# khimansusinha/Distributed-sorting-with-fault-tolerance

Measured on AMD Instinct MI355X. Metric: sorted keys/sec (int32, 2^30 keys), higher is better.
Workload: dtype int32; 1 GPU; C2-style single-GPU sort of 1073741824 uniform int32 keys (BASELINE metric size); tile 8192 keys, 0 merge passes; keys=1073741824, parallelism=1 GPU

## Files before the change

### distributed-sorting-with-fault-tolerance_amd/csrc/dsort_internal.h

```cpp
#pragma once

#include <hip/hip_runtime.h>
#include <stdint.h>
#include <stddef.h>

#include <atomic>
#include <mutex>
#include <string>
#include <utility>
#include <vector>

#include "dsort.h"

struct ncclComm;
namespace dsort {
class TxSeq;
}

namespace dsort {

constexpr int kMaxLogF = 5;
constexpr int kMaxF = 1 << kMaxLogF;

struct GroupK {
// ... 79 lines not shown
    void mark_at(int i, hipStream_t s) {
        if (!ok || i >= kMax) return;
        ok = (ev[i].h || hipEventCreate(&ev[i].h) == hipSuccess) && hipEventRecord(ev[i], s) == hipSuccess;
        if (ok) n = i + 1;
    }
    int count() const { return ok ? n : 0; }
    bool complete(int events) const { return count() == events; }
    int wait_last(dsort_ctx *ctx) const;
    int elapsed(dsort_ctx *ctx, int a, int b, double *ms) const;
};

}

struct dsort_opts {
    int64_t buckets = -1;
    int64_t bucket_keys = 1 << 20;
    static constexpr int64_t BUCKET_OS_DEFAULT = 128;
    int64_t bucket_os = BUCKET_OS_DEFAULT;
    int64_t max_logf = -1;
    int64_t kill_after_pass = -1;
    int64_t stage_timing = 1;
    int64_t kill_in_exchange = -1;
    int64_t comm_timeout_ms = 0;
    int64_t test_hold_exchange = 0;
    int64_t test_fail_exchange = -1;
    int64_t test_tile_cap = 0;
    int64_t test_wave_fence = 0;
    int64_t sub_keys = -1;
    int64_t sub_os = -1;
    int64_t sub_gather = 1;
    int64_t argsort_wide = 0;
    int64_t test_fail_leg = -1;
    int64_t topk_path = -1;
};

struct dsort_ctx {
    using DevBuf = dsort::DevBuf;
    using HostBuf = dsort::HostBuf;
    using Event = dsort::Event;
    using Stream = dsort::Stream;
    using LegClock = dsort::LegClock;

    dsort_opts opt;
    int nested = 0;
    int stages_done = 0;
    std::atomic<int> abort_req{0};
    std::mutex comm_mu;
    int device = 0;
    std::string err;

    Stream stream;
    Stream side;
    Stream xs;

    Event groups_ev;
    Event bucket_ev;
    Event sub_ev;
    Event side_ev;
    Event ready_ev;
    Event done_ev;
    Event a64_mm_ev;
    Event xev[3];
    Event ev[dsort::kStageEvents];
    static constexpr int kMaxKev = 128;
    Event kev[kMaxKev];
    LegClock pairs_clk;
// ... 37 lines not shown
    DevBuf gat_rep;
    DevBuf gat_back;
    DevBuf gat_small;
    HostBuf gat_host;
    DevBuf bucket;
    HostBuf bucket_host;
    DevBuf sub;
    DevBuf sub_alt;
    DevBuf stmp;
    HostBuf sub_host;
    hipStream_t done_stream = nullptr;
    bool done_pending = false;
    DevBuf tfb;
    DevBuf text_status;
    DevBuf red;
    HostBuf red_host;
    ncclComm *comm = nullptr;
    bool has_transport = false;
    dsort_transport transport = {};
    dsort::TxSeq *tx = nullptr;
    HostBuf xfer;
    HostBuf xfer2;
    DevBuf fence;
    HostBuf fence_host;
    int nranks = 1;
    int rank = 0;
    DevBuf local;
    DevBuf recv;
    DevBuf recv2;
    DevBuf small;
    HostBuf small_host;
    DevBuf bxs;
    const uint32_t *bk_hot = nullptr;
    int ev_off = 0;
    int ev_done = dsort::kEvLocalDone;
    bool poll_waits = false;
    double poll_deadline = 0.0;
    hipStream_t poll_stream = nullptr;
    std::vector<void *> dev_later, host_later;
    uint64_t deferred_n = 0;
    unsigned ev_mask = 0;
    hipStream_t last_stream = nullptr;
    int kev_used = 0;
    bool ev_ok = false;
    bool ev_created = false;
    dsort_stats stats = {};
};

namespace dsort {

__device__ __forceinline__ uint32_t wave_incl_sum(uint32_t v) {
    v += (uint32_t)__builtin_amdgcn_update_dpp(0, (int)v, 0x111, 0xF, 0xF, false);
    v += (uint32_t)__builtin_amdgcn_update_dpp(0, (int)v, 0x112, 0xF, 0xF, false);
    v += (uint32_t)__builtin_amdgcn_update_dpp(0, (int)v, 0x114, 0xF, 0xF, false);
    v += (uint32_t)__builtin_amdgcn_update_dpp(0, (int)v, 0x118, 0xF, 0xF, false);
    v += (uint32_t)__builtin_amdgcn_update_dpp(0, (int)v, 0x142, 0xA, 0xF, false);
    v += (uint32_t)__builtin_amdgcn_update_dpp(0, (int)v, 0x143, 0xC, 0xF, false);
    return v;
}

inline dsort_stats fresh_stats() {
    dsort_stats s{};
    s.first_level_map = -1;
    return s;
}

// ... 73 lines not shown
```

### distributed-sorting-with-fault-tolerance_amd/csrc/dsort_sub.h

```cpp
#pragma once
#include <hip/hip_runtime.h>
#include <stdint.h>

#include "dsort_bucket.h"

namespace dsort {
namespace sb {

constexpr int SB_T = 256;
constexpr int SB_MAXS = 1024;
constexpr int SB_SLOTB = 10;
constexpr int SB_SLOTS = 1 << SB_SLOTB;
constexpr int SB_ST = 4;
template <typename T> constexpr int SB_KPT = sizeof(T) == 4 ? 16 : 8;
template <typename T> constexpr int SB_SUB = SB_T * SB_KPT<T>;
template <typename T> constexpr int SB_CH = SB_ST * SB_SUB<T>;

struct BInfo {
    uint64_t start;
    uint64_t soff;
    uint32_t len;
    uint32_t nsub;
    uint32_t ns;
    uint32_t c0, c1;
// ... 6 lines not shown
    uint32_t len;
    uint32_t b;
    uint32_t boff;
    uint32_t pad;
};

__device__ __forceinline__ uint64_t bucket_src_pos(const BInfo &b, const Chunk *ch, uint64_t p) {
    if (!b.multi) return b.start + p;
    uint32_t lo = b.c0, hi = b.c1 - 1;
    while (lo < hi) {
        const uint32_t mid = (lo + hi + 1) >> 1;
        if (ch[mid].boff <= p) lo = mid;
        else hi = mid - 1;
    }
    return ch[lo].start + (p - ch[lo].boff);
}

template <typename T>
__device__ __forceinline__ Chunk chunk_of(const Chunk *ch, const BInfo *bi, uint32_t c) {
    if (ch) return ch[c];
    const uint64_t o = (uint64_t)c * SB_CH<T>, len = bi[0].len;
    return Chunk{bi[0].start + o, (uint32_t)(len - o < (uint64_t)SB_CH<T> ? len - o : (uint64_t)SB_CH<T>), 0u,
                 (uint32_t)o, 0u};
}

template <typename T> struct KeyU;
template <> struct KeyU<int32_t> { using U = uint32_t; };
template <> struct KeyU<int64_t> { using U = uint64_t; };

template <typename T>
struct SlotFn {
    T klo;
    uint32_t sh;
    uint32_t pad;
};

template <typename T>
__host__ __device__ __forceinline__ uint32_t slot_of(T key, T klo, uint32_t sh) {
    using U = typename KeyU<T>::U;
    const U d = key < klo ? (U)0 : (U)((U)key - (U)klo);
    const U s = d >> sh;
    return s > (U)(SB_SLOTS - 1) ? (uint32_t)(SB_SLOTS - 1) : (uint32_t)s;
}

template <typename T> struct Spl;
template <> struct __attribute__((aligned(8))) Spl<int32_t> {
    int32_t k;
    uint32_t p;
};
template <> struct __attribute__((aligned(16))) Spl<int64_t> {
    int64_t k;
    uint32_t p, pad;
};

template <typename T>
__device__ __forceinline__ bool below(const Spl<T> &s, T key, uint32_t pos) {
    return s.k < key || (s.k == key && s.p <= pos);
}

constexpr uint32_t SB_ONEKEY = 0x8000u;
template <typename T>
__device__ __forceinline__ int sub_pick(const Spl<T> *spl, uint32_t r, const Spl<T> &a, const Spl<T> &b, T key,
                                        uint32_t pos) {
    int lo = (int)(r & 0x7FFF);
    const int hi = (int)(r >> 16);
    if (r & SB_ONEKEY) {
        if (key != a.k) return key < a.k ? lo : hi;
        if (pos < a.p) return lo;
        const Spl<T> z = spl[hi - 1];
        if (pos >= z.p) return hi;
        const float f = (float)((pos * 2654435761u) >> 8) * 0x1p-24f;
        const int jj = (int)(f * (float)(hi - lo - 1));
        return lo + 1 + (jj < hi - lo - 2 ? jj : hi - lo - 2);
    }
    const int j = lo + (lo < hi && below<T>(a, key, pos) ? 1 + (lo + 1 < hi && below<T>(b, key, pos)) : 0);
    if (j < lo + 2 || j >= hi) return j;
    lo = j;
    int h = hi;
    while (lo < h) {
        const int mid = (lo + h) >> 1;
        if (below<T>(spl[mid], key, pos)) lo = mid + 1;
        else h = mid;
    }
    return lo;
}
template <typename T>
__device__ __forceinline__ int sub_of(const Spl<T> *spl, const uint32_t *rng, T klo, uint32_t sh, T key,
                                      uint32_t pos) {
    const uint32_t r = rng[slot_of<T>(key, klo, sh)];
    const int lo = (int)(r & 0x7FFF), hi = (int)(r >> 16);
    Spl<T> a{}, b{};
    if (lo < hi) a = spl[lo];
    if (lo + 1 < hi) b = spl[lo + 1];
    return sub_pick<T>(spl, r, a, b, key, pos);
}

constexpr uint32_t SB_RUN = 8;
constexpr uint32_t SB_SMP_CH = 1024;
__host__ __device__ __forceinline__ uint32_t sample_run(const BInfo &b) { return b.single || b.ns % SB_RUN ? 1u : SB_RUN; }
__host__ __device__ __forceinline__ uint64_t sample_run_pos(const BInfo &b, uint32_t run, uint64_t r) {
    const uint64_t nr = b.ns / run;
    const uint64_t p = ((2 * r + 1) * b.len) / (2 * nr);
    return p + run > b.len ? b.len - run : p;
}
__host__ __device__ __forceinline__ uint64_t sample_pos(const BInfo &b, uint64_t k) {
    const uint32_t run = sample_run(b);
    return sample_run_pos(b, run, k / run) + k % run;
}
template <typename T>
__global__ void __launch_bounds__(SB_T) sb_sample_kernel(const T *__restrict__ src, const BInfo *__restrict__ bi,
                                                         const Chunk *__restrict__ ch, T *__restrict__ smp,
                                                         int64_t *__restrict__ cmp) {
    const BInfo b = bi[blockIdx.x];
    auto put = [&](uint64_t k, T key) {
        const uint64_t g = b.soff + k;
        smp[g] = key;
        if constexpr (sizeof(T) == 4) cmp[g] = (int64_t)((uint64_t)(int64_t)key << 32 | (uint32_t)g);
    };
    if (sample_run(b) == SB_RUN && !b.multi) {
#pragma unroll 2
// ... 39 lines not shown

template <typename T>
__device__ __forceinline__ uint32_t lower_bound_k(const T *a, uint32_t n, T k) {
    uint32_t lo = 0, hi = n;
    while (lo < hi) {
        const uint32_t mid = (lo + hi) >> 1;
        if (a[mid] < k) lo = mid + 1;
        else hi = mid;
    }
    return lo;
}
template <typename T>
__device__ __forceinline__ uint32_t upper_bound_k(const T *a, uint32_t n, T k) {
    uint32_t lo = 0, hi = n;
    while (lo < hi) {
        const uint32_t mid = (lo + hi) >> 1;
        if (!(k < a[mid])) lo = mid + 1;
        else hi = mid;
    }
    return lo;
}

__global__ void __launch_bounds__(SB_T) sb_rank_kernel(const int64_t *__restrict__ smp, const int64_t *__restrict__ srt,
                                                       const BInfo *__restrict__ bi, int64_t *__restrict__ cmp) {
    const BInfo b = bi[blockIdx.x];
    for (uint32_t k = threadIdx.x; k < b.ns; k += SB_T) {
        const uint64_t g = b.soff + k;
        const uint64_t lo = b.soff + lower_bound_k<int64_t>(srt + b.soff, b.ns, smp[g]);
        cmp[g] = (int64_t)(lo << 32 | (uint32_t)g);
    }
}

template <typename T>
__global__ void __launch_bounds__(SB_MAXS) sb_splitter_kernel(const int64_t *__restrict__ cmp, const T *__restrict__ smp,
                                                              const BInfo *__restrict__ bi, const Chunk *__restrict__ ch,
                                                              int os, int SS,
                                                              Spl<T> *__restrict__ spl, uint32_t *__restrict__ rng,
                                                              SlotFn<T> *__restrict__ sfn, uint32_t *__restrict__ stot) {
    using U = typename KeyU<T>::U;
    __shared__ uint32_t sslot[SB_MAXS];
    __shared__ T skey[SB_MAXS];
    const BInfo b = bi[blockIdx.x];
    const int tid = threadIdx.x;
    if (stot)
        for (int j = tid; j < SS; j += SB_MAXS) stot[(uint64_t)blockIdx.x * SS + j] = 0;
    const int nspl = (int)b.nsub - 1;
    T klo = 0;
    uint32_t sh = 0;
    if (nspl > 0) {
        const int64_t *cm = cmp + b.soff;
        klo = smp[(uint32_t)cm[0]];
        const U span = (U)((U)smp[(uint32_t)cm[b.ns - 1]] - (U)klo);
        while (sh < 8 * sizeof(T) && (span >> sh) >= (U)SB_SLOTS) ++sh;
        if (tid < nspl) {
            const uint32_t g = (uint32_t)cm[(uint32_t)(tid + 1) * (uint32_t)os - 1];
            const T K = smp[g];
            Spl<T> sp{};
            sp.k = K;
            sp.p = (uint32_t)bucket_src_pos(b, ch, sample_pos(b, g - b.soff));
            spl[(uint64_t)blockIdx.x * SS + tid] = sp;
            sslot[tid] = slot_of<T>(K, klo, sh);
            skey[tid] = K;
        }
    }
    __syncthreads();
    for (int s = tid; s < SB_SLOTS; s += SB_MAXS) {
        uint32_t lo = 0, hi = (uint32_t)(nspl > 0 ? nspl : 0);
        while (lo < hi) {
            const uint32_t mid = (lo + hi) >> 1;
            if (sslot[mid] < (uint32_t)s) lo = mid + 1;
            else hi = mid;
        }
        uint32_t lo2 = lo, hi2 = (uint32_t)(nspl > 0 ? nspl : 0);
        while (lo2 < hi2) {
            const uint32_t mid = (lo2 + hi2) >> 1;
            if (sslot[mid] <= (uint32_t)s) lo2 = mid + 1;
            else hi2 = mid;
        }
        const bool one = lo2 >= lo + 3 && skey[lo] == skey[lo2 - 1];
        rng[(uint64_t)blockIdx.x * SB_SLOTS + s] = lo | (one ? SB_ONEKEY : 0u) | (lo2 << 16);
    }
    if (tid == 0) sfn[blockIdx.x] = SlotFn<T>{klo, sh, 0};
}

template <typename T>
__device__ __forceinline__ void load_sub_tables(const BInfo &b, uint32_t bid, int SS, const Spl<T> *spl_g,
                                                const uint32_t *rng_g, Spl<T> *spl, uint32_t *rng) {
    const int nspl = (int)b.nsub - 1;
    for (int j = threadIdx.x; j < nspl; j += blockDim.x) spl[j] = spl_g[(uint64_t)bid * SS + j];
    for (int s = threadIdx.x; s < SB_SLOTS; s += blockDim.x) rng[s] = rng_g[(uint64_t)bid * SB_SLOTS + s];
}

template <typename T>
__global__ void __launch_bounds__(SB_T) sb_hist_kernel(const T *__restrict__ src, const Chunk *__restrict__ ch,
                                                       const BInfo *__restrict__ bi, int SS,
                                                       const Spl<T> *__restrict__ spl_g,
                                                       const uint32_t *__restrict__ rng_g,
                                                       const SlotFn<T> *__restrict__ sfn,
                                                       uint32_t *__restrict__ counts) {
    __shared__ Spl<T> spl[SB_MAXS + 1];
    __shared__ uint32_t rng[SB_SLOTS];
    __shared__ uint32_t hist[SB_MAXS];
    const Chunk c = chunk_of<T>(ch, bi, blockIdx.x);
    const BInfo b = bi[c.b];
    uint32_t *out = counts + (uint64_t)blockIdx.x * SS;
    if (b.nsub == 1) {
        if (threadIdx.x == 0) out[0] = c.len;
        return;
    }
    load_sub_tables<T>(b, c.b, SS, spl_g, rng_g, spl, rng);
    for (int j = threadIdx.x; j < (int)b.nsub; j += SB_T) hist[j] = 0;
    const SlotFn<T> f = sfn[c.b];
    __syncthreads();
    constexpr int UN = 8;
#pragma unroll 1
// ... 375 lines not shown
#define SBST(k)                                            \
    do {                                                   \
        const uint64_t t1_ = __builtin_amdgcn_s_memtime(); \
        st_acc[k] = t1_ - st_t0;                           \
        st_t0 = t1_;                                       \
    } while (0)
#else
#define SBST(k) \
    do {        \
    } while (0)
#endif
    const uint32_t cid = sb_chunk_order(blockIdx.x, gridDim.x);
    const Chunk c = ch[cid];
    const BInfo b = bi[c.b];
    uint32_t *pc = pref + (uint64_t)cid * (SS + 1);
    const int tid = threadIdx.x, lane = tid & 63, w = tid >> 6;
    const int ns = (int)b.nsub;
    if (ns == 1) {
        if (tid == 0) {
            pc[0] = 0;
            pc[1] = c.len;
            if (stot) atomicAdd(&stot[(uint64_t)c.b * SS], c.len);
        }
        return;
    }
    const uint32_t m = 0;
    T *src = buf + c.start;
    T key[KPT];
#pragma unroll
    for (int k = 0; k < KPT; ++k) {
        const uint32_t s = tid + k * LT;
        key[k] = s - m < c.len ? src[s] : T(0);
    }
    load_sub_tables<T>(b, c.b, SS, spl_g, rng_g, spl, rng);
#pragma unroll
    for (int q = 0; q < PER; ++q) hist[PER * tid + q] = 0;
    const SlotFn<T> f = sfn[c.b];
    const bool hotf = hotp != nullptr && *hotp != 0;
    __syncthreads();
    SBST(0);
    uint32_t pk[KPT];
    constexpr int G = sizeof(T) == 4 ? SB_G32 : SB_G64;
    const bool whole = c.len == (uint32_t)CHL;
    if constexpr (G == 1) {
        if (hotf) {
#pragma unroll
            for (int k = 0; k < KPT; ++k) {
                const uint32_t s = tid + k * LT;
                const bool act = s - m < c.len;
                const int j = act ? sub_of<T>(spl, rng, f.klo, f.sh, key[k], (uint32_t)(c.start + s - m)) : 0;
                pk[k] = (uint32_t)j | bk::bucket_bump<true>(hist, j, act) << 10;
            }
        } else if (whole) {
#pragma unroll
            for (int k = 0; k < KPT; ++k) {
                const uint32_t s = tid + k * LT;
                if ((k > 0 && k + 1 < KPT) || s - m < c.len) {
                    const int j = sub_of<T>(spl, rng, f.klo, f.sh, key[k], (uint32_t)(c.start + s - m));
                    pk[k] = (uint32_t)j | atomicAdd(&hist[j], 1u) << 10;
                }
            }
        } else
#pragma unroll
        for (int k = 0; k < KPT; ++k) {
            const uint32_t s = tid + k * LT;
            if (s - m < c.len) {
                const int j = sub_of<T>(spl, rng, f.klo, f.sh, key[k], (uint32_t)(c.start + s - m));
                pk[k] = (uint32_t)j | atomicAdd(&hist[j], 1u) << 10;
            }
        }
    } else {
#pragma unroll
    for (int g0 = 0; g0 < KPT; g0 += G) {
        uint32_t r[G];
        Spl<T> sa[G], sb[G];
#pragma unroll
        for (int u = 0; u < G; ++u)
// ... 170 lines not shown
```

### distributed-sorting-with-fault-tolerance_amd/csrc/dsort_wave.hip

```cpp
#include <hip/hip_runtime.h>

#include <stdint.h>

#include <algorithm>
#include <climits>
#include <ctime>
#include <sched.h>
#include <unistd.h>
#include <csignal>
#include <cstdlib>
#include <cstring>
#include <string>
#include <type_traits>
#include <vector>

#include "dsort_bucket.h"
#include "dsort_internal.h"
#include "dsort_tx.h"

#include <rocprofiler-sdk-roctx/roctx.h>
#include "dsort_part.h"
#include "dsort_sub.h"

namespace dsort {
// ... 1529 lines not shown
    uint32_t *rng;
    sb::SlotFn<T> *sfn;
    uint32_t *cnt, *offs;
    void *tt;
    sb::Ovf *ovf;
    uint32_t *num;
    bk::TileRef *stl;
    uint2 *pcs;
    FillSeg<T> *fill;
    uint32_t *stot;
    uint32_t *hn;
};
template <typename T>
static size_t sub_arena(const SubArgs<T> &a, const SubPlan<T> &p, uintptr_t base, SubArena<T> &A) {
    using namespace sb;
    const size_t B = (size_t)a.B, SS = (size_t)p.SS;
    uintptr_t at = base;
    auto take = [&](auto *&ptr, size_t bytes) {
        ptr = reinterpret_cast<std::remove_reference_t<decltype(ptr)>>(at);
        at += (bytes + 255) & ~(size_t)255;
    };
    take(A.bi, B * sizeof(BInfo));
    take(A.ch, p.nch * sizeof(Chunk));
    take(A.smp, p.nsmp * sizeof(T));
    take(A.cmp, p.nsmp * 8);
    take(A.srt, sizeof(T) == 8 ? p.nsmp * 8 : 0);
    take(A.spl, B * SS * sizeof(Spl<T>));
    take(A.rng, B * SB_SLOTS * 4);
    take(A.sfn, B * sizeof(SlotFn<T>));
    take(A.cnt, p.nch * (SS + 1) * 4);
    take(A.offs, p.local ? 0 : p.nch * SS * 4);
    take(A.tt, p.tmax * sizeof(GTile));
    take(A.ovf, p.nsubs * sizeof(Ovf));
    take(A.num, 8);
    take(A.stl, B * sizeof(bk::TileRef) + 16);
    take(A.pcs, p.local ? p.tcap * p.PS * sizeof(uint2) : 0);
    take(A.fill, a.pm || a.fill_keys ? B * sizeof(FillSeg<T>) : 0);
    take(A.stot, p.totals ? B * SS * 4 : 0);
    if (!p.totals) A.stot = nullptr;
    return at - base;
}

template <typename T>
static SubPlan<T> sub_plan(const dsort_opts &opt, const SubArgs<T> &a, uint64_t m_in, bool local, bool retry) {
    using namespace sb;
    const int B = a.B;
    const uint64_t *hb = a.hb;
    const uint8_t *pure = a.pure;
    const PieceMap<T> *pm = a.pm;
    SubPlan<T> p;
    uint64_t maxlen = 0;
    for (int b = 0; b < B; ++b)
        if (!pure[b]) maxlen = std::max<uint64_t>(maxlen, hb[b + 1] - hb[b]);
    const int TILE = sizeof(T) == 4 && maxlen > (uint64_t)SB_MAXS * TILE_OF<T> / 4 ? TILE_W<16> : TILE_OF<T>;
    const uint64_t m = opt.sub_keys < 0 && TILE != TILE_OF<T> ? (uint64_t)TILE / 8 : m_in;
    constexpr uint64_t ALIGN = KPC<T>;
    const bool asked_local = local;
    const uint64_t LCH = SB_LCH<T>;
    auto bucket_chunks = [&](int b, uint64_t ch) -> uint64_t {
        if (pure[b]) return 0;
        if (!pm) return ceil_div(hb[b + 1] - hb[b], ch);
        uint64_t c = 0;
        for (uint32_t q = pm->first[b]; q < pm->first[b + 1]; ++q) c += ceil_div(pm->p[q].len, ch);
        return c;
    };
    for (int b = 0; b < B && local; ++b)
        if (bucket_chunks(b, LCH) > (uint64_t)kMaxPieces<T>) local = false;
// ... 80 lines not shown
        release_host(ctx, ctx->sub_host);
        DSORT_HIP(ctx, hipHostMalloc(&ctx->sub_host.p, hbytes, hipHostMallocDefault));
        ctx->sub_host.bytes = hbytes;
    }
    char *h = ctx->sub_host.as<char>();
    A.hn = reinterpret_cast<uint32_t *>(h + h_num);
    std::memcpy(h, bi.data(), B * sizeof(BInfo));
    Chunk *hc = reinterpret_cast<Chunk *>(h + h_ch);
    for (size_t b = 0; b < B; ++b) {
        if (!bi[b].len) continue;
        if (!pm) {
            for (uint64_t o = 0; o < bi[b].len; o += CH)
                *hc++ = Chunk{bi[b].start + o, (uint32_t)(bi[b].len - o < CH ? bi[b].len - o : CH), (uint32_t)b,
                              (uint32_t)o, 0u};
            continue;
        }
        uint64_t boff = 0;
        for (uint32_t q = pm->first[b]; q < pm->first[b + 1]; ++q) {
            const SrcPiece &pc = pm->p[q];
            for (uint64_t o = 0; o < pc.len; o += CH, boff += CH)
                *hc++ = Chunk{pc.src + o, (uint32_t)(pc.len - o < CH ? pc.len - o : CH), (uint32_t)b, (uint32_t)boff, 0u};
            boff -= ceil_div(pc.len, CH) * CH - pc.len;
        }
    }
    const size_t nfill = p.fill.size(), nst = p.stl.size();
    if (nfill) std::memcpy(h + h_fill, p.fill.data(), nfill * sizeof(FillSeg<T>));
    bk::TileRef *hst = reinterpret_cast<bk::TileRef *>(h + h_stl);
    if (nst) std::memcpy(hst, p.stl.data(), nst * sizeof(bk::TileRef));
    *reinterpret_cast<uint32_t *>(hst + B) = (uint32_t)nst;
    if ((rc = side_stream(ctx))) return rc;
    DSORT_HIP(ctx, hipMemcpyAsync(A.bi, h, B * sizeof(BInfo), hipMemcpyHostToDevice, ctx->side));
    if (nch) DSORT_HIP(ctx, hipMemcpyAsync(A.ch, h + h_ch, nch * sizeof(Chunk), hipMemcpyHostToDevice, ctx->side));
    DSORT_HIP(ctx, hipMemcpyAsync(A.stl, hst, B * sizeof(bk::TileRef) + 16, hipMemcpyHostToDevice, ctx->side));
    DSORT_HIP(ctx, hipMemsetAsync(A.num, 0, 8, ctx->side));
    if (nfill)
        DSORT_HIP(ctx, hipMemcpyAsync(A.fill, h + h_fill, nfill * sizeof(FillSeg<T>), hipMemcpyHostToDevice, ctx->side));
    DSORT_HIP(ctx, hipEventRecord(ctx->side_ev, ctx->side));
    DSORT_HIP(ctx, hipStreamWaitEvent(a.s, ctx->side_ev, 0));
    ctx->stats.tile_sort_keys = a.n - p.npure;
    return DSORT_OK;
}

template <typename T>
static int sub_splitters(dsort_ctx *ctx, const SubArgs<T> &a, const SubPlan<T> &p, const SubArena<T> &A) {
    using namespace sb;
    const int B = a.B;
    const uint64_t *hb = a.hb;
    const uint8_t *pure = a.pure;
    hipStream_t s = a.s;
    int rc;
    if (const uint32_t nfill = (uint32_t)p.fill.size()) {
        const unsigned gx = (unsigned)std::min<uint64_t>(ceil_div(p.maxfill, 256 * FILL_U * (16 / sizeof(T))), 1024);
        hipLaunchKernelGGL(fill_segments_kernel<T>, dim3(gx, nfill), dim3(256), 0, s, a.d_keys,
                           static_cast<const FillSeg<T> *>(A.fill));
        DSORT_HIP(ctx, hipGetLastError());
    }
    for (int b = 0; b < B && !a.pure_done && !a.pm;) {
        if (!pure[b]) {
            ++b;
            continue;
        }
        int e = b;
        while (e < B && pure[e]) ++e;
        if (hb[e] > hb[b])
            DSORT_HIP(ctx, hipMemcpyAsync(a.d_keys + hb[b], a.src + hb[b], (hb[e] - hb[b]) * sizeof(T),
                                          hipMemcpyDeviceToDevice, s));
        b = e;
    }
    if (p.nsmp) {
        const uint32_t nst = (uint32_t)p.stl.size();
        hipLaunchKernelGGL(sb_sample_kernel<T>, dim3((unsigned)B), dim3(SB_T), 0, s, a.src, A.bi, A.ch, A.smp, A.cmp);
        DSORT_HIP(ctx, hipGetLastError());
        const uint4 *stl4 = reinterpret_cast<const uint4 *>(A.stl);
        const uint32_t *pnst = reinterpret_cast<const uint32_t *>(A.stl + B);
        if constexpr (sizeof(T) == 8) {
            rc = tile_sort<int64_t, false>(ctx, A.smp, A.srt, p.nsmp, stl4, pnst, sb::Gather{}, nst, s, false);
            if (rc) return rc;
            hipLaunchKernelGGL(sb_rank_kernel, dim3((unsigned)B), dim3(SB_T), 0, s, A.smp, A.srt, A.bi, A.cmp);
        }
        rc = tile_sort<int64_t, false>(ctx, A.cmp, A.cmp, p.nsmp, stl4, pnst, sb::Gather{}, nst, s, false);
        if (rc) return rc;
        hipLaunchKernelGGL(sb_splitter_kernel<T>, dim3((unsigned)B), dim3(SB_MAXS), 0, s, A.cmp, A.smp, A.bi, A.ch, p.os,
                           p.SS, A.spl, A.rng, A.sfn, A.stot);
        DSORT_HIP(ctx, hipGetLastError());
    } else if (A.stot) {
        DSORT_HIP(ctx, hipMemsetAsync(A.stot, 0, (size_t)B * p.SS * 4, s));
    }
    return DSORT_OK;
}

template <typename T>
static int sub_local_path(dsort_ctx *ctx, const SubArgs<T> &a, const SubPlan<T> &p, const SubArena<T> &A,
                          bool &overflow) {
    using namespace sb;
    constexpr uint64_t ALIGN = KPC<T>;
    const int B = a.B, TILE = p.TILE, SS = p.SS;
    const uint64_t n = a.n, tcap = p.tcap;
    const uint32_t PS = p.PS;
    T *src = a.src, *d_keys = a.d_keys;
    hipStream_t s = a.s;
    const bool timed = a.timed;
    uint32_t *num = A.num;
    int rc;
    if (p.nch) {
        if ((rc = stage_event(ctx, s, timed, wave_ev(ctx, kEvSub0)))) return rc;
        hipLaunchKernelGGL(sb_local_kernel<T>, dim3((unsigned)p.nch), dim3(SB_LT<T>), 0, s, src, A.ch, A.bi, SS, A.spl,
                           A.rng, A.sfn, A.cnt, ctx->bk_hot, A.stot);
        DSORT_HIP(ctx, hipGetLastError());
        if ((rc = stage_event(ctx, s, timed, wave_ev(ctx, kEvSub1)))) return rc;
    }
    constexpr int PIECES_SCAN_MINB = 256;
    const bool pieces_in_scan = B >= PIECES_SCAN_MINB;
    hipLaunchKernelGGL(sb_scan_kernel<true>, dim3((unsigned)B), dim3(SB_MAXS), 0, s, A.bi, SS, A.cnt, nullptr, TILE, 1,
                       0u, (uint32_t)(2 * (ALIGN - 1)), A.tt, num, A.ovf, num + 1, (uint32_t)p.tmax,
                       static_cast<const Chunk *>(A.ch), pieces_in_scan ? A.pcs : nullptr, PS, (uint32_t)tcap, A.stot);
    DSORT_HIP(ctx, hipGetLastError());
    const GTile *gtiles = static_cast<const GTile *>(A.tt);
    const Gather ga{gtiles, A.ch, A.bi, A.cnt, A.pcs, PS, SS, A.spl, a.bspl, B, (uint32_t)std::max<uint64_t>(tcap, 1)};
    const bool pieces_early = !pieces_in_scan && A.pcs && tcap > 0;
    if (pieces_early) {
        hipLaunchKernelGGL(sb_pieces_kernel, dim3((unsigned)ceil_div(tcap, 4)), dim3(256), 0, s, gtiles, num,
                           static_cast<const Chunk *>(A.ch), A.cnt, SS, A.pcs, PS, (uint32_t)tcap);
        DSORT_HIP(ctx, hipGetLastError());
    }
    DSORT_HIP(ctx, hipMemcpyAsync(A.hn, num, 8, hipMemcpyDeviceToHost, s));
    DSORT_HIP(ctx, hipEventRecord(ctx->sub_ev, s));
    const uint64_t ebound = (n - p.npure) / (uint64_t)TILE;
    const uint32_t early = (pieces_in_scan || pieces_early) && ctx->opt.kill_after_pass != 1
                               ? (uint32_t)std::min<uint64_t>(ebound, tcap)
                               : 0u;
    if (early) {
        if ((rc = tile_sort_event(ctx, s, timed, 0))) return rc;
        rc = with_tile_waves<T>(ctx, TILE, [&](auto w) {
            return tile_sort_begin<T, true, decltype(w)::value>(ctx, src, d_keys, n, nullptr, num, ga, early,
                                                                (uint32_t)tcap, s);
        });
        if (rc) return rc;
    }
    if (int rc_ = sync_event(ctx, ctx->sub_ev, "tile count")) return rc_;
    const uint32_t ntiles = A.hn[0], novf = A.hn[1];
    if (ntiles > p.tmax || ntiles > tcap) {
        if (early)
            if (int rc_ = sync_stream(ctx, s, "early tile sort")) return rc_;
        ctx->stats.sub_scatter_fallback = 1;
        overflow = true;
        return DSORT_OK;
    }
    if (ntiles && !pieces_in_scan && !pieces_early) {
        hipLaunchKernelGGL(sb_pieces_kernel, dim3((unsigned)ceil_div(ntiles, 4)), dim3(256), 0, s, gtiles, num,
                           static_cast<const Chunk *>(A.ch), A.cnt, SS, A.pcs, PS, (uint32_t)tcap);
        DSORT_HIP(ctx, hipGetLastError());
    }
    fault_point(ctx, s, 1);
    ctx->stats.merge_passes = 0;
    if (early) {
        rc = with_tile_waves<T>(ctx, TILE, [&](auto w) {
            constexpr int W = decltype(w)::value;
            int r = tile_sort_more<T, true, W>(ctx, src, d_keys, n, nullptr, num, ga, early,
                                               ntiles > early ? ntiles - early : 0u, (uint32_t)tcap, s);
            return r ? r : tile_sort_end<T, true, W>(ctx, src, d_keys, n, nullptr, num, ga, ntiles, (uint32_t)tcap, s);
        });
        if (rc) return rc;
        if ((rc = tile_sort_event(ctx, s, timed, 1))) return rc;
    } else if (ntiles) {
        rc = tile_sort<T, true>(ctx, src, d_keys, n, nullptr, num, ga, ntiles, s, timed, TILE);
        if (rc) return rc;
    }
    if ((rc = stage_event(ctx, s, timed, wave_ev(ctx, kEvTileSortDone)))) return rc;
    fault_point(ctx, s, 2);
    if (novf) {
        rc = merge_split_subbuckets<T>(ctx, A.ovf, novf, gtiles, d_keys, s);
        if (rc) return rc;
    }
    return sort_done_event(ctx, s, timed);
}

template <typename T>
static int sub_scatter_path(dsort_ctx *ctx, const SubArgs<T> &a, const SubPlan<T> &p, const SubArena<T> &A) {
    using namespace sb;
    constexpr uint64_t ALIGN = KPC<T>;
    const int B = a.B, TILE = p.TILE, SS = p.SS;
    const uint64_t nch = p.nch;
    T *src = a.src, *d_keys = a.d_keys;
    hipStream_t s = a.s;
    const bool timed = a.timed;
    uint32_t *num = A.num;
    const uint32_t mis = (uint32_t)((reinterpret_cast<uintptr_t>(d_keys) / sizeof(T)) & (ALIGN - 1));
    int rc;
    if (nch) {
        if ((rc = stage_event(ctx, s, timed, wave_ev(ctx, kEvSub0)))) return rc;
        hipLaunchKernelGGL(sb_hist_kernel<T>, dim3((unsigned)nch), dim3(SB_T), 0, s, src, A.ch, A.bi, SS, A.spl, A.rng,
                           A.sfn, A.cnt);
        DSORT_HIP(ctx, hipGetLastError());
    }
    hipLaunchKernelGGL(sb_scan_kernel<false>, dim3((unsigned)B), dim3(SB_MAXS), 0, s, A.bi, SS, A.cnt, A.offs, TILE,
                       (int)ALIGN, mis, 0u, A.tt, num, A.ovf, num + 1, (uint32_t)p.tmax, nullptr, nullptr, 0u, 0u, nullptr);
    DSORT_HIP(ctx, hipGetLastError());
    DSORT_HIP(ctx, hipMemcpyAsync(A.hn, num, 8, hipMemcpyDeviceToHost, s));
    DSORT_HIP(ctx, hipEventRecord(ctx->sub_ev, s));
    if (nch) {
        hipLaunchKernelGGL(sb_scatter_kernel<T>, dim3((unsigned)nch), dim3(SB_T), 0, s, src, d_keys, A.ch,
                           (uint32_t)nch, A.bi, SS, A.spl, A.rng, A.sfn, A.offs);
        DSORT_HIP(ctx, hipGetLastError());
        if ((rc = stage_event(ctx, s, timed, wave_ev(ctx, kEvSub1)))) return rc;
    }
    if (int rc_ = sync_event(ctx, ctx->sub_ev, "tile count")) return rc_;
    const uint32_t ntiles = A.hn[0], novf = A.hn[1];
    if (ntiles > p.tmax || novf > p.nsubs) return set_err(ctx, DSORT_EHIP, "sub-bucket packing overflow");
    fault_point(ctx, s, 1);
    ctx->stats.merge_passes = 0;
    if (ntiles) {
        rc = tile_sort<T, false>(ctx, d_keys, d_keys, a.n, static_cast<const uint4 *>(A.tt), num, Gather{}, ntiles, s,
                                 timed, TILE);
        if (rc) return rc;
    }
    if ((rc = stage_event(ctx, s, timed, kEvTileSortDone))) return rc;
    fault_point(ctx, s, 2);
    if (novf) {
        std::vector<Ovf> ov(novf);
        DSORT_HIP(ctx, hipMemcpyAsync(ov.data(), A.ovf, novf * sizeof(Ovf), hipMemcpyDeviceToHost, s));
        if (int rc_ = sync_stream(ctx, s, "sort stream")) return rc_;
        uint64_t mx = 0;
        for (const Ovf &o : ov) mx = o.len > mx ? o.len : mx;
        if (int rc_ = ensure(ctx, ctx->stmp, mx * sizeof(T) + 16, "oversized sub-bucket merge"))
            return rc_;
        T *tmp = ctx->stmp.as<T>();
        int lv = 0;
        for (const Ovf &o : ov) {
            const std::vector<size_t> runs = sub_tile_runs(o.start, o.len, TILE, ALIGN, mis);
            T *to = tmp + ((o.start + mis) & (ALIGN - 1));
            rc = wave_merge<T>(ctx, d_keys + o.start, runs.data(), (int)runs.size(), to, s, true);
            if (rc) return rc;
            DSORT_HIP(ctx, hipMemcpyAsync(d_keys + o.start, to, o.len * sizeof(T), hipMemcpyDeviceToDevice, s));
            int l = 0;
            for (uint64_t r = runs.size(); r > 1; r = ceil_div(r, (uint64_t)1 << WG<T>::MAXLOGF)) ++l;
            lv = l > lv ? l : lv;
        }
        ctx->stats.merge_passes = lv;
        ctx->stats.sub_split_subbuckets = (int)novf;
    }
    return sort_done_event(ctx, s, timed);
// ... 121 lines not shown
    DSORT_HIP(ctx, hipStreamWaitEvent(ctx->side, ctx->ready_ev, 0));
    DSORT_HIP(ctx, hipMemcpyAsync(hb, L.bst, (size_t)(B + 1) * 8, hipMemcpyDeviceToHost, ctx->side));
    if (B > 1) DSORT_HIP(ctx, hipMemcpyAsync(hspl, L.spl, (size_t)(B - 1) * sizeof(C), hipMemcpyDeviceToHost, ctx->side));
    DSORT_HIP(ctx, hipEventRecord(ctx->bucket_ev, ctx->side));
    if ((rc = stage_event(ctx, s, timed, kEvScatter0))) return rc;
    if constexpr (!Comp<T>::ADAPT) {
        if (ad)
            hipLaunchKernelGGL((bucket_scatter_lines_kernel<T, false, true>), dim3((unsigned)L.G), dim3(BK_T), 0, s,
                               d_in, n, L.spl, L.map, B, BP, L.subs, L.offs, part_out, direct, ioff, L.ids);
    }
    if (!ad && !ids) {
        if (!Comp<T>::ADAPT && hm->hot)
            hipLaunchKernelGGL((bucket_scatter_lines_kernel<T, false, false, true>), dim3((unsigned)L.G), dim3(BK_T), 0,
                               s, d_in, n, L.spl, L.map, B, BP, L.subs, L.offs, part_out, direct, ioff, L.ids);
        else
            hipLaunchKernelGGL((bucket_scatter_lines_kernel<T, false, false>), dim3((unsigned)L.G), dim3(BK_T), 0, s,
                               d_in, n, L.spl, L.map, B, BP, L.subs, L.offs, part_out, direct, ioff, L.ids);
    }
    if constexpr (BkIds<T>::ON)
        if (ids)
            hipLaunchKernelGGL((bucket_scatter_lines_kernel<T, true>), dim3((unsigned)L.G), dim3(BK_T), 0, s, d_in, n,
                               L.spl, L.map, B, BP, L.subs, L.offs, part_out, direct, ioff, L.ids);
    DSORT_HIP(ctx, hipGetLastError());
    if ((rc = stage_event(ctx, s, timed, kEvScatter1))) return rc;
    fault_point(ctx, s, 0);
    if (int rc_ = sync_event(ctx, ctx->bucket_ev, "bucket starts")) return rc_;
    if (hb[B] != n) return set_err(ctx, DSORT_EHIP, "bucket partition lost keys");
    ctx->stats.first_level_map = !Comp<T>::ADAPT && !ad ? (hm->r2s ? 3 : 0) : hm->mode == 0 ? 1 : 2;
    return DSORT_OK;
}

static int bucketed_stats_start(dsort_ctx *ctx, uint64_t n, int tile, hipStream_t s, bool timed) {
    ctx->bk_hot = nullptr;
    ctx->stats = fresh_stats();
    ctx->stats.keys_in = ctx->stats.keys_out = n;
    ctx->stats.tile_sort_keys = n;
    ctx->stats.tile_keys = tile;
    ctx->ev_mask = 0;
    ctx->kev_used = 0;
    ctx->last_stream = s;
    return stage_event(ctx, s, timed, kEvStart);
}

template <typename T>
static int bucket_sort(dsort_ctx *ctx, const T *d_in, T *d_keys, size_t n, hipStream_t s, bool timed, int B) {
    using namespace bk;
    using C = typename Comp<T>::C;
    constexpr int TILE = TILE_OF<T>;
    constexpr uint64_t ALIGN = KPC<T>;
    const int os = bucket_os(ctx);
    const uint32_t S = (uint32_t)B * (uint32_t)os;
    BkLayout<T> L;
    int rc = bk_layout<T>(ctx, n, B, (size_t)S * (sizeof(T) == 8 ? 24 : sizeof(C)), L);
    if (rc) return rc;
    const int BP = L.BP;
    C *smp = reinterpret_cast<C *>(L.smp);
    C *spl = L.spl;
    TileRef *tt = L.tt;
    uint32_t *ntl = L.ntl;
    const uint64_t tmax = L.tmax;
    rc = ensure(ctx, ctx->scratch, n * sizeof(T) + 16, "sort scratch");
    if (rc) return rc;
    T *scratch = ctx->scratch.as<T>();
    int64_t *pk = reinterpret_cast<int64_t *>(smp), *psrt = pk + S, *pcmp = pk + 2 * (size_t)S;
    ++ctx->nested;
    if constexpr (std::is_same<T, int32_t>::value) {
// ... 525 lines not shown
            GroupK &gk = gh[gi];
            gk.base = base;
            gk.first_tile = tiles;
            gk.nruns = 0;
            gk.pad = 0;
            uint64_t tot = 0;
            gk.roff[0] = 0;
            for (int r = gi * MAXF; r < nr && r < (gi + 1) * MAXF; ++r) {
                tot += rl[r];
                gk.roff[++gk.nruns] = tot;
            }
            for (int r = (int)gk.nruns + 1; r <= kMaxF; ++r) gk.roff[r] = tot;
            gk.total = tot;
            tiles += ceil_div(tot, MTN);
            base += tot;
            next.push_back(tot);
        }
        DSORT_HIP(ctx, hipMemcpyAsync(ctx->groups.p, gh, gbytes, hipMemcpyHostToDevice, s));
        DSORT_HIP(ctx, hipEventRecord(ctx->groups_ev, s));
        ctx->groups_ev_pending = true;
        PassDesc pd{n, 0, 1 << logf, ng, ctx->groups.as<const GroupK>()};
        T *dst = dsts[which];
        rc = launch_pass_w<T, false>(ctx, src, dst, pd, logf, tiles, s, !keep_stats);
        if (rc) return rc;
        rl.swap(next);
        src = dst;
        which ^= 1;
    }
    return DSORT_OK;
}

}

#ifdef DSORT_STAMPS
extern "C" int dsort_debug_stamps(void *host, size_t bytes) {
    return hipMemcpyFromSymbol(host, HIP_SYMBOL(wv::g_stamps), bytes) == hipSuccess ? 0 : -1;
}
extern "C" int dsort_debug_bkstamps(void *host, size_t bytes) {
    return hipMemcpyFromSymbol(host, HIP_SYMBOL(bk::g_bkstamps), bytes) == hipSuccess ? 0 : -1;
}
extern "C" int dsort_debug_sbstamps(void *host, size_t bytes) {
    return hipMemcpyFromSymbol(host, HIP_SYMBOL(sb::g_sbstamps), bytes) == hipSuccess ? 0 : -1;
}
#endif

void PollPause::operator()() {
    const double t = tx_now_ms();
    if (t0 < 0) t0 = t;
    if (t - t0 < POLL_SPIN_MS) sched_yield();
    else usleep(20);
}
static int poll_done(dsort_ctx *ctx, hipError_t (*query)(void *), void *h, const char *what, bool comm) {
    PollPause pause;
    for (;;) {
        const hipError_t q = query(h);
        if (q == hipSuccess) return DSORT_OK;
        if (q != hipErrorNotReady) return hip_err(ctx, q, what);
        if (comm && ctx->abort_req.load())
            return set_err(ctx, DSORT_ECOMM, std::string(what) + ": aborted by dsort_comm_abort (keys in flight)");
        if (comm && ctx->poll_deadline > 0 && tx_now_ms() > ctx->poll_deadline)
            return set_err(ctx, DSORT_ETIMEOUT, std::string(what) + ": no progress before the deadline (keys in flight)");
        pause();
    }
}
int sync_event(dsort_ctx *ctx, hipEvent_t e, const char *what) {
    return poll_done(ctx, [](void *h) { return hipEventQuery(static_cast<hipEvent_t>(h)); }, e, what, ctx->poll_waits);
// ... 81 lines not shown
```

### distributed-sorting-with-fault-tolerance_amd/dsort.py

```python
import contextlib
import ctypes
import os

import numpy as np

HERE = os.path.dirname(os.path.abspath(__file__))
LIB_PATH = os.environ.get("DSORT_LIB") or os.path.join(HERE, "lib", "libdsort.so")

try:
    import torch
except Exception:
    torch = None

DSORT_OK = 0
DSORT_ECOMM = -4
DSORT_ETIMEOUT = -6
ERRORS = {-1: "EINVAL", -2: "ENOMEM", -3: "EHIP", -4: "ECOMM", -5: "ENODEV", -6: "ETIMEOUT", -7: "ESTAGE"}

EXPORTS = [
    "dsort_init", "dsort_finalize", "dsort_last_error", "dsort_version", "dsort_get_stats",
    "dsort_synchronize", "dsort_set_option", "dsort_get_option", "dsort_sort_stages", "dsort_sample_sort_stages", "dsort_sort_i32", "dsort_sort_i64", "dsort_sort_dev_i32",
    "dsort_sort_dev_i64", "dsort_sort_dev_copy_i32", "dsort_sort_dev_copy_i64",
    "dsort_merge_i32", "dsort_merge_i64", "dsort_merge_dev_i32", "dsort_merge_dev_i64",
    "dsort_comm_unique_id", "dsort_comm_init", "dsort_comm_init_transport", "dsort_comm_abort",
# ... 428 lines not shown

    def close(self):
        if self.h:
            self.lib.dsort_finalize(self.h)
            self.h = None

    def __enter__(self):
        return self

    def __exit__(self, *exc):
        self.close()

    def __del__(self):
        try:
            self.close()
        except Exception:
            pass

    def check(self, rc):
        return _check(self.h, rc)

    @staticmethod
    def _opt(name):
        return OPTIONS[name]

    def set_option(self, name, value):
        self.check(self.lib.dsort_set_option(self.h, self._opt(name), int(value)))

    def get_option(self, name):
        v = ctypes.c_int64()
        self.check(self.lib.dsort_get_option(self.h, self._opt(name), ctypes.byref(v)))
        return v.value

    @contextlib.contextmanager
    def options(self, **kw):
        old = {k: self.get_option(k) for k in kw}
        try:
            for k, v in kw.items():
                self.set_option(k, v)
            yield self
        finally:
            for k, v in old.items():
                self.set_option(k, v)

    def sort_stages(self, n, key_bytes=4):
        m = ctypes.c_int()
        self.check(self.lib.dsort_sort_stages(self.h, n, key_bytes, ctypes.byref(m)))
        return m.value

    def sort(self, keys, descending=False, key_type=None):
        assert keys.flags.c_contiguous
        name = _np_key(keys, key_type)
        if name in ("i32", "i64") and not descending:
            f = getattr(self.lib, f"dsort_sort_{name}")
            self.check(f(self.h, _ptr(keys), keys.size))
        else:
            self.check(self.lib.dsort_sort_keys(self.h, _ptr(keys), keys.size, KEY_TYPES[name],
                                                ORDER_DESCENDING if descending else 0))
        return keys

    def merge(self, runs):
        runs = [np.ascontiguousarray(r) for r in runs]
        dt = runs[0].dtype if runs else np.dtype(np.int32)
        k = len(runs)
        ptrs = (ctypes.c_void_p * max(k, 1))(*[r.ctypes.data for r in runs])
        lens = (ctypes.c_size_t * max(k, 1))(*[r.size for r in runs])
# ... 408 lines not shown
```

Before: 143.2 billion keys/s.

## Use arithmetic equal-width sub-bucket splitters for int32 when samples are uniform

For 32-bit keys, the splitter kernel now tries evenly spaced key ranges computed from the sample span. It validates them against the sorted samples, rejecting them if any sub-bucket would be too large. When accepted, the scatter kernel computes each key's sub-bucket with a multiply-shift instead of a slot table lookup plus binary search over splitters. It also skips loading the splitter tables into shared memory. The cost is an extra shared-memory validation pass in the splitter kernel, and a risk of skewed sub-bucket sizes, which the bounded-size check is meant to catch.

```diff
diff --git a/distributed-sorting-with-fault-tolerance_amd/csrc/dsort_internal.h b/distributed-sorting-with-fault-tolerance_amd/csrc/dsort_internal.h
--- a/distributed-sorting-with-fault-tolerance_amd/csrc/dsort_internal.h
+++ b/distributed-sorting-with-fault-tolerance_amd/csrc/dsort_internal.h
@@ -135,6 +135,7 @@
     int64_t argsort_wide = 0;
     int64_t test_fail_leg = -1;
     int64_t topk_path = -1;
+    int64_t sub_arith = -1;
 };
 
 struct dsort_ctx {
@@ -238,6 +239,7 @@
     HostBuf small_host;
     DevBuf bxs;
     const uint32_t *bk_hot = nullptr;
+    uint32_t sub_arith_n[2] = {0, 0};
     int ev_off = 0;
     int ev_done = dsort::kEvLocalDone;
     bool poll_waits = false;
diff --git a/distributed-sorting-with-fault-tolerance_amd/csrc/dsort_sub.h b/distributed-sorting-with-fault-tolerance_amd/csrc/dsort_sub.h
--- a/distributed-sorting-with-fault-tolerance_amd/csrc/dsort_sub.h
+++ b/distributed-sorting-with-fault-tolerance_amd/csrc/dsort_sub.h
@@ -62,7 +62,7 @@
 struct SlotFn {
     T klo;
     uint32_t sh;
-    uint32_t pad;
+    uint32_t scale;
 };
 
 template <typename T>
@@ -83,14 +83,32 @@
     uint32_t p, pad;
 };
 
-template <typename T>
-__device__ __forceinline__ bool below(const Spl<T> &s, T key, uint32_t pos) {
+template <typename T> constexpr bool SB_ARITH = sizeof(T) == 4;
+__host__ __device__ __forceinline__ bool arith_span_ok(uint32_t span, uint32_t nsub) { return span >= 2 * nsub; }
+__host__ __device__ __forceinline__ uint32_t arith_scale(uint32_t span, uint32_t nsub) {
+    return (uint32_t)(((uint64_t)nsub << 32) / ((uint64_t)span + 1));
+}
+__host__ __device__ __forceinline__ uint32_t arith_sub(int32_t key, int32_t klo, uint32_t scale, uint32_t nsub) {
+    const uint32_t d = key < klo ? 0u : (uint32_t)key - (uint32_t)klo;
+    const uint32_t j = (uint32_t)(((uint64_t)d * scale) >> 32);
+    return j < nsub - 1 ? j : nsub - 1;
+}
+__host__ __device__ __forceinline__ int32_t arith_splitter_key(int32_t klo, uint32_t scale, uint32_t j) {
+    const uint64_t d = ((((uint64_t)j + 1) << 32) + scale - 1) / scale - 1;
+    const int64_t k = (int64_t)klo + (int64_t)d;
+    return k < (int64_t)INT32_MAX ? (int32_t)k : INT32_MAX;
+}
+constexpr uint32_t SB_ARITH_MAXS = 3;
+constexpr uint32_t SB_ARITH_MAXS_RUNS = 6;
+
+template <typename T>
+__host__ __device__ __forceinline__ bool below(const Spl<T> &s, T key, uint32_t pos) {
     return s.k < key || (s.k == key && s.p <= pos);
 }
 
 constexpr uint32_t SB_ONEKEY = 0x8000u;
 template <typename T>
-__device__ __forceinline__ int sub_pick(const Spl<T> *spl, uint32_t r, const Spl<T> &a, const Spl<T> &b, T key,
+__host__ __device__ __forceinline__ int sub_pick(const Spl<T> *spl, uint32_t r, const Spl<T> &a, const Spl<T> &b, T key,
                                         uint32_t pos) {
     int lo = (int)(r & 0x7FFF);
     const int hi = (int)(r >> 16);
@@ -115,7 +133,7 @@
     return lo;
 }
 template <typename T>
-__device__ __forceinline__ int sub_of(const Spl<T> *spl, const uint32_t *rng, T klo, uint32_t sh, T key,
+__host__ __device__ __forceinline__ int sub_of(const Spl<T> *spl, const uint32_t *rng, T klo, uint32_t sh, T key,
                                       uint32_t pos) {
     const uint32_t r = rng[slot_of<T>(key, klo, sh)];
     const int lo = (int)(r & 0x7FFF), hi = (int)(r >> 16);
@@ -221,11 +239,37 @@
 }
 
 template <typename T>
+__host__ __device__ __forceinline__ uint32_t slot_entry(const uint32_t *sslot, const T *skey, uint32_t nspl, uint32_t s) {
+    uint32_t lo = 0, hi = nspl;
+    while (lo < hi) {
+        const uint32_t mid = (lo + hi) >> 1;
+        if (sslot[mid] < s) lo = mid + 1;
+        else hi = mid;
+    }
+    uint32_t lo2 = lo, hi2 = nspl;
+    while (lo2 < hi2) {
+        const uint32_t mid = (lo2 + hi2) >> 1;
+        if (sslot[mid] <= s) lo2 = mid + 1;
+        else hi2 = mid;
+    }
+    const bool one = lo2 >= lo + 3 && skey[lo] == skey[lo2 - 1];
+    return lo | (one ? SB_ONEKEY : 0u) | (lo2 << 16);
+}
+template <typename T>
+__host__ __device__ __forceinline__ uint32_t slot_shift(typename KeyU<T>::U span) {
+    using U = typename KeyU<T>::U;
+    uint32_t sh = 0;
+    while (sh < 8 * sizeof(T) && (span >> sh) >= (U)SB_SLOTS) ++sh;
+    return sh;
+}
+
+template <typename T>
 __global__ void __launch_bounds__(SB_MAXS) sb_splitter_kernel(const int64_t *__restrict__ cmp, const T *__restrict__ smp,
                                                               const BInfo *__restrict__ bi, const Chunk *__restrict__ ch,
                                                               int os, int SS,
                                                               Spl<T> *__restrict__ spl, uint32_t *__restrict__ rng,
-                                                              SlotFn<T> *__restrict__ sfn, uint32_t *__restrict__ stot) {
+                                                              SlotFn<T> *__restrict__ sfn, uint32_t *__restrict__ stot,
+                                                              int arith, uint32_t *__restrict__ actr) {
     using U = typename KeyU<T>::U;
     __shared__ uint32_t sslot[SB_MAXS];
     __shared__ T skey[SB_MAXS];
@@ -235,41 +279,63 @@
         for (int j = tid; j < SS; j += SB_MAXS) stot[(uint64_t)blockIdx.x * SS + j] = 0;
     const int nspl = (int)b.nsub - 1;
     T klo = 0;
-    uint32_t sh = 0;
+    uint32_t sh = 0, scale = 0;
     if (nspl > 0) {
         const int64_t *cm = cmp + b.soff;
         klo = smp[(uint32_t)cm[0]];
         const U span = (U)((U)smp[(uint32_t)cm[b.ns - 1]] - (U)klo);
-        while (sh < 8 * sizeof(T) && (span >> sh) >= (U)SB_SLOTS) ++sh;
+        sh = slot_shift<T>(span);
+        if constexpr (SB_ARITH<T>) {
+            constexpr uint32_t MAXNS = SB_MAXS * 8;
+            __shared__ int32_t sk[MAXNS];
+            __shared__ uint32_t bad, same;
+            if (arith != 0 && b.ns <= MAXNS && arith_span_ok((uint32_t)span, b.nsub)) {
+                scale = arith_scale((uint32_t)span, b.nsub);
+                if (arith < 0) {
+                    for (uint32_t i = tid; i < b.ns; i += SB_MAXS) sk[i] = (int32_t)(cm[i] >> 32);
+                    if (tid == 0) bad = same = 0;
+                    __syncthreads();
+                    if (const uint32_t run = sample_run(b); run > 1) {
+                        uint32_t n1 = 0;
+                        for (uint32_t i = tid + 1; i < b.ns; i += SB_MAXS)
+                            n1 += ((uint32_t)cm[i] - (uint32_t)b.soff) / run == ((uint32_t)cm[i - 1] - (uint32_t)b.soff) / run;
+                        if (n1) atomicAdd(&same, n1);
+                    }
+                    uint32_t ub = b.ns;
+                    if (tid < nspl) ub = upper_bound_k<int32_t>(sk, b.ns, arith_splitter_key(klo, scale, (uint32_t)tid));
+                    if (tid <= nspl) sslot[tid] = ub;
+                    __syncthreads();
+                    const uint32_t maxs = 2 * same >= b.ns ? SB_ARITH_MAXS_RUNS : SB_ARITH_MAXS;
+                    if (tid <= nspl && ub - (tid ? sslot[tid - 1] : 0u) > maxs * (uint32_t)os) bad = 1;
+                    __syncthreads();
+                    if (bad) scale = 0;
+                    __syncthreads();
+                }
+            }
+        }
         if (tid < nspl) {
-            const uint32_t g = (uint32_t)cm[(uint32_t)(tid + 1) * (uint32_t)os - 1];
-            const T K = smp[g];
             Spl<T> sp{};
-            sp.k = K;
-            sp.p = (uint32_t)bucket_src_pos(b, ch, sample_pos(b, g - b.soff));
+            if (SB_ARITH<T> && scale) {
+                if constexpr (SB_ARITH<T>) sp.k = arith_splitter_key(klo, scale, (uint32_t)tid);
+                sp.p = UINT32_MAX;
+            } else {
+                const uint32_t g = (uint32_t)cm[(uint32_t)(tid + 1) * (uint32_t)os - 1];
+                sp.k = smp[g];
+                sp.p = (uint32_t)bucket_src_pos(b, ch, sample_pos(b, g - b.soff));
+            }
             spl[(uint64_t)blockIdx.x * SS + tid] = sp;
-            sslot[tid] = slot_of<T>(K, klo, sh);
-            skey[tid] = K;
-        }
-    }
-    __syncthreads();
-    for (int s = tid; s < SB_SLOTS; s += SB_MAXS) {
-        uint32_t lo = 0, hi = (uint32_t)(nspl > 0 ? nspl : 0);
-        while (lo < hi) {
-            const uint32_t mid = (lo + hi) >> 1;
-            if (sslot[mid] < (uint32_t)s) lo = mid + 1;
-            else hi = mid;
-        }
-        uint32_t lo2 = lo, hi2 = (uint32_t)(nspl > 0 ? nspl : 0);
-        while (lo2 < hi2) {
-            const uint32_t mid = (lo2 + hi2) >> 1;
-            if (sslot[mid] <= (uint32_t)s) lo2 = mid + 1;
-            else hi2 = mid;
-        }
-        const bool one = lo2 >= lo + 3 && skey[lo] == skey[lo2 - 1];
-        rng[(uint64_t)blockIdx.x * SB_SLOTS + s] = lo | (one ? SB_ONEKEY : 0u) | (lo2 << 16);
-    }
-    if (tid == 0) sfn[blockIdx.x] = SlotFn<T>{klo, sh, 0};
+            sslot[tid] = slot_of<T>(sp.k, klo, sh);
+            skey[tid] = sp.k;
+        }
+        if (tid == 0 && actr) {
+            atomicAdd(&actr[0], 1u);
+            if (scale) atomicAdd(&actr[1], 1u);
+        }
+    }
+    __syncthreads();
+    for (int s = tid; s < SB_SLOTS; s += SB_MAXS)
+        rng[(uint64_t)blockIdx.x * SB_SLOTS + s] = slot_entry<T>(sslot, skey, (uint32_t)(nspl > 0 ? nspl : 0), (uint32_t)s);
+    if (tid == 0) sfn[blockIdx.x] = SlotFn<T>{klo, sh, scale};
 }
 
 template <typename T>
@@ -711,17 +777,49 @@
         const uint32_t s = tid + k * LT;
         key[k] = s - m < c.len ? src[s] : T(0);
     }
-    load_sub_tables<T>(b, c.b, SS, spl_g, rng_g, spl, rng);
+    const SlotFn<T> f = sfn[c.b];
+    bool arith = false;
+    if constexpr (SB_ARITH<T>) arith = f.scale != 0;
+    if (!arith) load_sub_tables<T>(b, c.b, SS, spl_g, rng_g, spl, rng);
 #pragma unroll
     for (int q = 0; q < PER; ++q) hist[PER * tid + q] = 0;
-    const SlotFn<T> f = sfn[c.b];
     const bool hotf = hotp != nullptr && *hotp != 0;
     __syncthreads();
     SBST(0);
     uint32_t pk[KPT];
     constexpr int G = sizeof(T) == 4 ? SB_G32 : SB_G64;
     const bool whole = c.len == (uint32_t)CHL;
-    if constexpr (G == 1) {
+    if (arith) {
+        if constexpr (SB_ARITH<T>) {
+            uint32_t jv[KPT];
+#pragma unroll
+            for (int k = 0; k < KPT; ++k) jv[k] = arith_sub(key[k], f.klo, f.scale, (uint32_t)ns);
+            if (hotf) {
+#pragma unroll
+                for (int k = 0; k < KPT; ++k) {
+                    const uint32_t s = tid + k * LT;
+                    pk[k] = jv[k] | bk::bucket_bump<true>(hist, (int)jv[k], s - m < c.len) << 10;
+                }
+            } else {
+                uint32_t rk[KPT];
+                if (whole) {
+#pragma unroll
+                    for (int k = 0; k < KPT; ++k) {
+                        const bool act = (k > 0 && k + 1 < KPT) || (uint32_t)(tid + k * LT) - m < c.len;
+                        rk[k] = atomicAdd(&hist[act ? jv[k] : (uint32_t)lane], act ? 1u : 0u);
+                    }
+                } else {
+#pragma unroll
+                    for (int k = 0; k < KPT; ++k) {
+                        const bool act = (uint32_t)(tid + k * LT) - m < c.len;
+                        rk[k] = atomicAdd(&hist[act ? jv[k] : (uint32_t)lane], act ? 1u : 0u);
+                    }
+                }
+#pragma unroll
+                for (int k = 0; k < KPT; ++k) pk[k] = jv[k] | rk[k] << 10;
+            }
+        }
+    } else if constexpr (G == 1) {
         if (hotf) {
 #pragma unroll
             for (int k = 0; k < KPT; ++k) {
diff --git a/distributed-sorting-with-fault-tolerance_amd/csrc/dsort_wave.hip b/distributed-sorting-with-fault-tolerance_amd/csrc/dsort_wave.hip
--- a/distributed-sorting-with-fault-tolerance_amd/csrc/dsort_wave.hip
+++ b/distributed-sorting-with-fault-tolerance_amd/csrc/dsort_wave.hip
@@ -1585,7 +1585,7 @@
     take(A.offs, p.local ? 0 : p.nch * SS * 4);
     take(A.tt, p.tmax * sizeof(GTile));
     take(A.ovf, p.nsubs * sizeof(Ovf));
-    take(A.num, 8);
+    take(A.num, 16);
     take(A.stl, B * sizeof(bk::TileRef) + 16);
     take(A.pcs, p.local ? p.tcap * p.PS * sizeof(uint2) : 0);
     take(A.fill, a.pm || a.fill_keys ? B * sizeof(FillSeg<T>) : 0);
@@ -1732,7 +1732,7 @@
     DSORT_HIP(ctx, hipMemcpyAsync(A.bi, h, B * sizeof(BInfo), hipMemcpyHostToDevice, ctx->side));
     if (nch) DSORT_HIP(ctx, hipMemcpyAsync(A.ch, h + h_ch, nch * sizeof(Chunk), hipMemcpyHostToDevice, ctx->side));
     DSORT_HIP(ctx, hipMemcpyAsync(A.stl, hst, B * sizeof(bk::TileRef) + 16, hipMemcpyHostToDevice, ctx->side));
-    DSORT_HIP(ctx, hipMemsetAsync(A.num, 0, 8, ctx->side));
+    DSORT_HIP(ctx, hipMemsetAsync(A.num, 0, 16, ctx->side));
     if (nfill)
         DSORT_HIP(ctx, hipMemcpyAsync(A.fill, h + h_fill, nfill * sizeof(FillSeg<T>), hipMemcpyHostToDevice, ctx->side));
     DSORT_HIP(ctx, hipEventRecord(ctx->side_ev, ctx->side));
@@ -1781,7 +1781,7 @@
         rc = tile_sort<int64_t, false>(ctx, A.cmp, A.cmp, p.nsmp, stl4, pnst, sb::Gather{}, nst, s, false);
         if (rc) return rc;
         hipLaunchKernelGGL(sb_splitter_kernel<T>, dim3((unsigned)B), dim3(SB_MAXS), 0, s, A.cmp, A.smp, A.bi, A.ch, p.os,
-                           p.SS, A.spl, A.rng, A.sfn, A.stot);
+                           p.SS, A.spl, A.rng, A.sfn, A.stot, (int)ctx->opt.sub_arith, A.num + 2);
         DSORT_HIP(ctx, hipGetLastError());
     } else if (A.stot) {
         DSORT_HIP(ctx, hipMemsetAsync(A.stot, 0, (size_t)B * p.SS * 4, s));
@@ -1823,7 +1823,7 @@
                            static_cast<const Chunk *>(A.ch), A.cnt, SS, A.pcs, PS, (uint32_t)tcap);
         DSORT_HIP(ctx, hipGetLastError());
     }
-    DSORT_HIP(ctx, hipMemcpyAsync(A.hn, num, 8, hipMemcpyDeviceToHost, s));
+    DSORT_HIP(ctx, hipMemcpyAsync(A.hn, num, 16, hipMemcpyDeviceToHost, s));
     DSORT_HIP(ctx, hipEventRecord(ctx->sub_ev, s));
     const uint64_t ebound = (n - p.npure) / (uint64_t)TILE;
     const uint32_t early = (pieces_in_scan || pieces_early) && ctx->opt.kill_after_pass != 1
@@ -1846,6 +1846,8 @@
         overflow = true;
         return DSORT_OK;
     }
+    ctx->sub_arith_n[0] += A.hn[2];
+    ctx->sub_arith_n[1] += A.hn[3];
     if (ntiles && !pieces_in_scan && !pieces_early) {
         hipLaunchKernelGGL(sb_pieces_kernel, dim3((unsigned)ceil_div(ntiles, 4)), dim3(256), 0, s, gtiles, num,
                            static_cast<const Chunk *>(A.ch), A.cnt, SS, A.pcs, PS, (uint32_t)tcap);
@@ -1896,7 +1898,7 @@
     hipLaunchKernelGGL(sb_scan_kernel<false>, dim3((unsigned)B), dim3(SB_MAXS), 0, s, A.bi, SS, A.cnt, A.offs, TILE,
                        (int)ALIGN, mis, 0u, A.tt, num, A.ovf, num + 1, (uint32_t)p.tmax, nullptr, nullptr, 0u, 0u, nullptr);
     DSORT_HIP(ctx, hipGetLastError());
-    DSORT_HIP(ctx, hipMemcpyAsync(A.hn, num, 8, hipMemcpyDeviceToHost, s));
+    DSORT_HIP(ctx, hipMemcpyAsync(A.hn, num, 16, hipMemcpyDeviceToHost, s));
     DSORT_HIP(ctx, hipEventRecord(ctx->sub_ev, s));
     if (nch) {
         hipLaunchKernelGGL(sb_scatter_kernel<T>, dim3((unsigned)nch), dim3(SB_T), 0, s, src, d_keys, A.ch,
@@ -1907,6 +1909,8 @@
     if (int rc_ = sync_event(ctx, ctx->sub_ev, "tile count")) return rc_;
     const uint32_t ntiles = A.hn[0], novf = A.hn[1];
     if (ntiles > p.tmax || novf > p.nsubs) return set_err(ctx, DSORT_EHIP, "sub-bucket packing overflow");
+    ctx->sub_arith_n[0] += A.hn[2];
+    ctx->sub_arith_n[1] += A.hn[3];
     fault_point(ctx, s, 1);
     ctx->stats.merge_passes = 0;
     if (ntiles) {
@@ -2094,6 +2098,7 @@
 
 static int bucketed_stats_start(dsort_ctx *ctx, uint64_t n, int tile, hipStream_t s, bool timed) {
     ctx->bk_hot = nullptr;
+    ctx->sub_arith_n[0] = ctx->sub_arith_n[1] = 0;
     ctx->stats = fresh_stats();
     ctx->stats.keys_in = ctx->stats.keys_out = n;
     ctx->stats.tile_sort_keys = n;
@@ -2685,6 +2690,18 @@
 
 }
 
+extern "C" int dsort_debug_sub_arith_mode(dsort_ctx *ctx, int mode) {
+    if (!ctx || (mode != -1 && mode != 0 && mode != 2)) return DSORT_EINVAL;
+    ctx->opt.sub_arith = mode;
+    return DSORT_OK;
+}
+extern "C" int dsort_debug_sub_arith(const dsort_ctx *ctx, uint32_t out[2]) {
+    if (!ctx || !out) return DSORT_EINVAL;
+    out[0] = ctx->sub_arith_n[0];
+    out[1] = ctx->sub_arith_n[1];
+    return DSORT_OK;
+}
+
 #ifdef DSORT_STAMPS
 extern "C" int dsort_debug_stamps(void *host, size_t bytes) {
     return hipMemcpyFromSymbol(host, HIP_SYMBOL(wv::g_stamps), bytes) == hipSuccess ? 0 : -1;
diff --git a/distributed-sorting-with-fault-tolerance_amd/dsort.py b/distributed-sorting-with-fault-tolerance_amd/dsort.py
--- a/distributed-sorting-with-fault-tolerance_amd/dsort.py
+++ b/distributed-sorting-with-fault-tolerance_amd/dsort.py
@@ -484,6 +484,18 @@
         self.check(self.lib.dsort_get_option(self.h, self._opt(name), ctypes.byref(v)))
         return v.value
 
+    def sub_arith_mode(self, mode):
+        f = self.lib.dsort_debug_sub_arith_mode
+        f.restype, f.argtypes = ctypes.c_int, [P, ctypes.c_int]
+        self.check(f(self.h, int(mode)))
+
+    def sub_arith_counts(self):
+        out = (ctypes.c_uint32 * 2)()
+        f = self.lib.dsort_debug_sub_arith
+        f.restype, f.argtypes = ctypes.c_int, [P, P]
+        self.check(f(self.h, ctypes.cast(out, P)))
+        return int(out[0]), int(out[1])
+
     @contextlib.contextmanager
     def options(self, **kw):
         old = {k: self.get_option(k) for k in kw}
```

Result: faster. 148.9 billion keys/s (median of 6 runs) (+4.0%).
